# SeanNobel/speech-decoding

Measured on AMD Instinct MI355X. Metric: train segments/sec (Gwilliams2022 208ch x 360, top-10 retrieval acc alongside), higher is better.
Workload: dtype bf16; 1 GPU; Gwilliams2022-shaped MEG: 208 ch x 360 samples, 27 subjects, F=1024, batch 256/GPU, fwd+CLIP loss+top-k+bwd+Adam (BASELINE configs[1]); global_batch=256, seq_len=360, parallelism=dp1

## Files before the change

### include/sd_amd.h

```cpp
#ifndef SD_AMD_H
#define SD_AMD_H
#include <stddef.h>
#include <stdint.h>

#ifdef __cplusplus
extern "C" {
#endif

#define SDA_ABI_VERSION 4
#define SDA_ROW_PAD 16
#define SDA_CH_ALIGN 64

enum { SDA_F32 = 0, SDA_BF16 = 1, SDA_F16 = 2 };

enum { SDA_EPI_GELU = 1,
       SDA_EPI_GLU_BWD = 4,
       SDA_EPI_GLU = 2,
       SDA_CONV_SINGLE_TILE = 4096,
       SDA_CONV_PAIR_TILES = 8192,
       SDA_CONV_ONE_PER_CU = 32768,
       SDA_CONV_FLAT_TILES = 16384,
       SDA_CONV_FLAT_STAGGER = 1024,
       SDA_CONV_WIDE_TILES = 524288,
       SDA_CONV_WAVE_PRIO = 1048576,
// ... 113 lines not shown
int sda_glu_backward_colsum(const void* x, const void* dy, void* dx, float* colsum, float* scratch, int B, int T,
                            int Ch, int dtype, void* stream);
int sda_gelu_backward_colsum(const void* u, const void* dz, void* du, float* colsum, float* scratch, int B, int T,
                             int Cp, int dtype, void* stream);
int sda_glu_backward_colsum_og(const void* out, const void* gate, const void* dy, void* dx, float* colsum, float* scratch,
                               int B, int T, int Ch, int dtype, void* stream);
int sda_colsum(const void* x, float* out, float* scratch , int B, int T,
               int Cp, int dtype, void* stream);

enum { SDA_WGRAD_FLAT_ROWS = 1   };
typedef struct sda_wgrad_args {
  const void* dy;
  const void* x;
  float* g;
  void* out_e;
  const void* sub;
  const float* rscale;
  const float* out_scale;
  const int32_t* perm;
  const int32_t* seg_start;
  int nseg, B, T, Cout_p, Cin_p, KS, dil;
  long dy_pitch, x_pitch, out_pitch;
  long row0, sample_rows;
  long rows_limit;
  long dy_zero_row;
  int co_valid;
  int dtype;
  const float* acc_scale;
  int flags;
} sda_wgrad_args;
int sda_wgrad_gemm(const sda_wgrad_args* a, void* stream);
int sda_wgrad_tile_m(int Cout_p);
int sda_reduce_slabs(const float* src, float* dst, int nslabs, long n, void* stream);
int sda_sim_gemm_ksplit(int M, int N, long K, int dtype);
int sda_sim_gemm(const void* X, const void* W, float* partial, int M, int N, int Np, long K, long pitch, int ksplit, int dtype,
                 void* stream);

int sda_sa_weights_forward(const float* z, const float* cos_t, const float* sin_t, const float* mask,
                           float* W, void* Wp, float* scratch , int D1, int K2,
                           int C, int D1p, int Cp, int dtype, void* stream);
int sda_sa_scratch_floats(int D1, int K2, int C);
int sda_sa_softmax_pack(const float* a, int a_pitch, const float* mask, float* W, void* Wp, int D1, int C, int D1p,
                        int Cp, int dtype, void* stream);
int sda_sa_softmax_backward(const float* dWd, int dwd_pitch, const float* W, const float* mask, float* da,
                            int da_pitch, int D1, int C, void* stream);
int sda_sa_weights_backward(const float* dWd, const float* W, const float* mask, const float* cosT,
                            const float* sinT, float* dz, int D1, int K2, int C, int Cp, void* stream);

int sda_clip_logits_stats(const float* S, long s_pitch, const float* ysq, const float* zsq, const float* temp,
                          float* logits, float* row_max, float* row_sum, float* col_lse, float* diag , float* row_lse ,
                          int Bm, int Bn, int col0, void* stream);
int sda_clip_grad(const float* logits, const float* row_lse, const float* col_lse, const float* ysq,
                  const float* zsq, const float* temp, float inv_norm, int col0, void* G, long g_pitch,
                  float* rscale, float* cscale, float* colpart, float* scalars, int Bm, int Bn, int dtype, void* stream);
int sda_clip_grad_y(const float* logits, const float* row_lse, const float* col_lse, const float* zsq,
                    const float* zsq_all, int nz, int col0, void* Gy, long gy_pitch, int seg, int seg_pitch,
                    float* part, int Bm, int Bn, int dtype, void* stream);
int sda_clip_grad_y_finish(const float* part, int nparts, int Bg, const float* ysq, const float* zsq_all, int nz,
                           const float* temp, float inv_norm, int row0, int nrows, float* rscale_y, float* cscale_y,
                           void* stream);
int sda_clip_dz_supported(int Bm, int Bn, long row_elems, int dtype);
int sda_clip_dz(const void* G, long g_pitch, const void* Y, const void* Z, void* out, const float* cscale, const float* rscale,
                const float* out_scale, int Bm, int Bn, long row_elems, int dtype, void* stream);
int sda_clip_ranks(const float* logits, const float* diag, int32_t* cnt, int Bm, int Bn, int col0, void* stream);
long sda_retrieval_scores_floats(int n, int M, int chunk_cols);
int sda_retrieval_select(const float* S, const float* qsq, const float* csq, const int64_t* labels, int64_t* indices,
// ... 79 lines not shown
```

### speech_decoding_amd/blocks.py

```python
from __future__ import annotations

from dataclasses import dataclass, field
from typing import Dict, Optional

import numpy as np
import torch

from . import lib as L
from . import ops
from .engine import block_dilations, subject_segments

FWD_FLAGS = L.CONV_PAIR_TILES
BWD_FLAGS = L.CONV_WAVE_PRIO


def rows_in(X: torch.Tensor, Cc: int, dtype):
    if X.dtype not in ops.COMPUTE_DTYPES:
        raise L.SdaError(f"input of dtype {X.dtype}: the modules take float32, bfloat16 or float16")
    return ops.rows_of(X, Cc, dtype, ops.new_rows_uninit)


def grad_rows(dY: torch.Tensor, Cc: int, dtype) -> torch.Tensor:
    return ops.rows_of(dY, Cc, dtype, ops.new_rows_uninit)[0]


def _new(B: int, T: int, Cp: int, dtype, dev) -> torch.Tensor:
    return ops.new_rows_uninit(B, T, Cp, dtype, dev)


def _segments(B: int, dy, x):
    nseg = ops.uniform_segment_count(B, ops.wgrad_ntiles(dy.shape[1], x.shape[1], 64))
    return ops.UPLOADER.upload("blocks.seg", ops.uniform_segment_edges(B, nseg), dy.device), nseg


def _wgrad(dy, x, B, T, KS, dil, Cout, Cin, glu_half=0, glu_half_p=0) -> torch.Tensor:
    seg, nseg = _segments(B, dy, x)
    slabs = ops.wgrad_gemm(dy, x, B=B, T=T, KS=KS, dil=dil, seg_start=seg, nseg=nseg, alg_dims=(Cin, Cout), flat_rows=True)
    return ops.reduce_unpack_wgrad(slabs, Cout, Cin, KS, glu_half=glu_half, glu_half_p=glu_half_p)


def _plans(module, dev, build):
    key = (str(dev), module.compute_dtype)
    plans = module.__dict__.setdefault("_block_plans", {})
# ... 59 lines not shown


def _sb_plans(sb):
    D1p = L.pad_channels(sb.D1)

    def build(f, b):
        f.add_weight("sb_w", sb.conv.weight, D1p, D1p)
        f.add_vector("sb_b", sb.conv.bias, D1p)
        f.add_weight("subj_w", sb.subject_layer.weight, D1p, D1p)
        b.add_weight("sb_w", sb.conv.weight, D1p, D1p, mode=1)
        b.add_weight("subj_w", sb.subject_layer.weight, D1p, D1p, mode=1)
        return f, b
    return _plans(sb, sb.conv.weight.device, build)


def _sb_sources(sb) -> Dict[str, torch.Tensor]:
    return {"sb_w": sb.conv.weight.detach(), "sb_b": sb.conv.bias.detach(), "subj_w": sb.subject_layer.weight.detach()}


def subject_block_forward(sb, X: torch.Tensor, sidx: np.ndarray, mask, need_grad: bool, want_subj_grad: bool):
    B, Cc, T = X.shape
    dt, dev, D1, S = sb.compute_dtype, X.device, sb.D1, sb.num_subjects
    D1p = L.pad_channels(D1)
    widx = ops.UPLOADER.upload("blocks.widx", sidx.astype(np.int32), dev)
    Xt, _ = rows_in(X, Cc, dt)
    h_sa, W, Wp = sa_forward(sb.spatial_attention, Xt, B, T, mask, dt)
    pk = _sb_plans(sb)[0].run(_sb_sources(sb))
    h_c = ops.conv_gemm(h_sa, pk["sb_w"], _new(B, T, D1p, dt, dev), B=B, T=T, KS=1, dil=0, bias=pk["sb_b"], alg_dims=(D1, D1))
    y = ops.conv_gemm(h_c, pk["subj_w"], _new(B, T, D1p, dt, dev), B=B, T=T, KS=1, dil=0, widx=widx, alg_dims=(D1, D1))
    if not need_grad:
        return y, None
    c = SBCtx(SACtx(B, T, Xt, W, Wp, mask, X.dtype), h_sa, h_c, widx)
    if want_subj_grad:
        r = ops.subject_slices(B, max(1, int(np.unique(sidx).size)), ops.wgrad_ntiles(D1p, D1p, 64))
        perm, seg = subject_segments(sidx, S, r)
        c.subj = (ops.UPLOADER.upload("blocks.subj_perm", perm, dev), ops.UPLOADER.upload("blocks.subj_seg", seg, dev), r)
    return y, c


def subject_block_backward(sb, c: SBCtx, dY: torch.Tensor, want: Dict[str, bool]) -> Dict[str, torch.Tensor]:
    _check_versions(c)
    B, T, dt, dev = c.sa.B, c.sa.T, sb.compute_dtype, dY.device
    D1, S = sb.D1, sb.num_subjects
    D1p = L.pad_channels(D1)
    g: Dict[str, torch.Tensor] = {}
    if want["subj_w"]:
        perm, seg, r = c.subj
        slabs = ops.wgrad_gemm(dY, c.h_c, B=B, T=T, KS=1, dil=0, perm=perm, seg_start=seg, nseg=r * S, flat_rows=True)
        if r > 1:
            slabs = ops.reduce_slabs(slabs.view(r, -1)).view(S, 1, D1p, D1p)
        g["subj_w"] = ops.unpack_conv_wgrad(slabs, S, D1, D1, 1, D1p, D1p)
    if not (want["sb_w"] or want["sb_b"] or want["z"] or want["X"]):
        return g
    pkT = _sb_plans(sb)[1].run(_sb_sources(sb))
    dh_c = ops.conv_gemm(dY, pkT["subj_w"], _new(B, T, D1p, dt, dev), B=B, T=T, KS=1, dil=0, widx=c.widx, alg_dims=(D1, D1),
                         flags=BWD_FLAGS)
    if want["sb_w"]:
        g["sb_w"] = _wgrad(dh_c, c.h_sa, B, T, 1, 0, D1, D1)
    if want["sb_b"]:
        g["sb_b"] = ops.colsum(dh_c, B, T, ops.reduce_scratch(D1p, dev))[:D1]
    if want["z"] or want["X"]:
        dh_sa = ops.conv_gemm(dh_c, pkT["sb_w"], _new(B, T, D1p, dt, dev), B=B, T=T, KS=1, dil=0, alg_dims=(D1, D1),
                              flags=BWD_FLAGS)
        g["X"], g["z"] = sa_backward(sb.spatial_attention, c.sa, dh_sa, want["X"], want["z"])
    return g


CB_PARAMS = ("c0w", "c0b", "bn0w", "bn0b", "c1w", "c1b", "bn1w", "bn1b", "c2w", "c2b")


def cb_params(cb):
    return [cb.conv0.weight, cb.conv0.bias, cb.batchnorm0.weight, cb.batchnorm0.bias, cb.conv1.weight, cb.conv1.bias,
            cb.batchnorm1.weight, cb.batchnorm1.bias, cb.conv2.weight, cb.conv2.bias]


@dataclass
class CBCtx:
    B: int
    T: int
    x: torch.Tensor
    x_rows: bool
    x_dtype: torch.dtype
    h: list
# ... 112 lines not shown
```

### speech_decoding_amd/csrc/elementwise.hip

```cpp
#include <math.h>

#include "sd_common.h"

namespace sda {

__device__ __forceinline__ void ew_bwd_prio() { __builtin_amdgcn_s_setprio(3); }

struct RowWalk {
  int r, r1, step, T, b, t;
  __device__ RowWalk(int r0, int r1_, int step_, int T_) : r(r0), r1(r1_), step(step_), T(T_) {
    b = r0 / T_;
    t = r0 - b * T_;
  }
  __device__ bool valid() const { return r < r1; }
  __device__ size_t mem_row() const { return (size_t)b * rows_tp(T) + PAD + t; }
  __device__ void next() {
    r += step; t += step;
    while (t >= T) { t -= T; ++b; }
  }
};

struct RowCursor {
  uint32_t off, step, wrap;
  int t, T, RG, n;
// ... 744 lines not shown
  const int RG = nch >= 256 ? 1 : 256 / nch;
  int r0, r1;
  block_rows(B, T, r0, r1);
  for (int c = threadIdx.x; c < RG * nch; c += 256) {
    const int ch = c % nch, rg = c / nch;
    for (RowWalk w(r0 + rg, r1, RG, T); w.valid(); w.next()) {
      const size_t off = w.mem_row() * Cp + ch * CH;
      float uv[CH], d[CH];
      Vec16<E>::load(u + off, uv);
      Vec16<E>::load(dz + off, d);
#pragma unroll
      for (int j = 0; j < CH; j += 2) {
        const f32x2 o = f32x2{d[j], d[j + 1]} * gelu_grad_pair<E>(f32x2{uv[j], uv[j + 1]});
        d[j] = o.x; d[j + 1] = o.y;
      }
      Vec16<E>::store(du + off, d);
    }
  }
}

__global__ void reduce_slabs_kernel(const float* __restrict__ src, float* __restrict__ dst, int nslabs, long n) {
  for (long i = (long)blockIdx.x * blockDim.x + threadIdx.x; i < n; i += (long)gridDim.x * blockDim.x) {
    float s = 0.f;
    int k = 0;
    for (; k + 8 <= nslabs; k += 8) {
      float v[8];
#pragma unroll
      for (int j = 0; j < 8; ++j) v[j] = src[(size_t)(k + j) * n + i];
#pragma unroll
      for (int j = 0; j < 8; ++j) s += v[j];
    }
    for (; k < nslabs; ++k) s += src[(size_t)k * n + i];
    dst[i] = s;
  }
}

static inline int ew_grid(size_t total) {
  size_t g = (total + 255) / 256;
  return (int)(g < 1 ? 1 : (g > 4096 ? 4096 : g));
}

static int red_blocks(int B, int T) {
  long rows = (long)B * T;
  long nb = (rows + 31) / 32;
  if (nb > RED_MAX_BLOCKS) nb = RED_MAX_BLOCKS;
  if (nb < 1) nb = 1;
  return (int)nb;
}

}

using namespace sda;

#define SDA_DISPATCH(dtype, CALL)                                   \
  do {                                                              \
    if ((dtype) == SDA_F32) { using E = float; CALL; }              \
    else if ((dtype) == SDA_BF16) { using E = uint16_t; CALL; }     \
    else if ((dtype) == SDA_F16) { using E = half_t; CALL; }        \
    else { set_error("unknown dtype %d", (int)(dtype)); return -1; } \
  } while (0)

namespace sda {
__global__ __launch_bounds__(256) void zero_pad_rows_kernel(uint4* __restrict__ buf, int B, int Tp, long rows_alloc, int row_vec) {
  const long pad_vecs = (long)B * PAD * row_vec, tail_vecs = (rows_alloc - (long)B * Tp) * row_vec;
  for (long i = (long)blockIdx.x * 256 + threadIdx.x; i < pad_vecs + tail_vecs; i += (long)gridDim.x * 256) {
    long v;
// ... 411 lines not shown
  hipStream_t st = (hipStream_t)stream;
  const int nb = red_blocks(B, T);
  const size_t lds = bwd_colsum_lds(Ch, dtype);
  SDA_DISPATCH(dtype, hipLaunchKernelGGL((bwd_colsum_kernel<E, 1>), dim3(nb), dim3(256), lds, st, (const E*)x,
                                         (const E*)dy, (E*)dx, scratch, B, T, Ch));
  if (colsum) hipLaunchKernelGGL(col_reduce_final_kernel, dim3((Ch + 7) / 8), dim3(256), 0, st, scratch, nb, colsum, colsum + Ch, Ch);
  return check_launch("glu_backward_colsum");
}

extern "C" int sda_glu_backward_colsum_og(const void* out, const void* gate, const void* dy, void* dx, float* colsum,
                                          float* scratch, int B, int T, int Ch, int dtype, void* stream) {
  if (!out || !gate || !dy || !dx || !scratch || Ch % 64 || Ch > 1024 || !fits_u32(B, T, 2L * Ch)) { set_error("glu_backward_colsum_og: bad arguments"); return -1; }
  hipStream_t st = (hipStream_t)stream;
  const int nb = red_blocks(B, T);
  const size_t lds = bwd_colsum_lds(Ch, dtype);
  SDA_DISPATCH(dtype, hipLaunchKernelGGL((bwd_colsum_kernel<E, 2>), dim3(nb), dim3(256), lds, st, (const E*)out,
                                         (const E*)dy, (E*)dx, scratch, B, T, Ch, (const E*)gate));
  if (colsum) hipLaunchKernelGGL(col_reduce_final_kernel, dim3((Ch + 7) / 8), dim3(256), 0, st, scratch, nb, colsum, colsum + Ch, Ch);
  return check_launch("glu_backward_colsum_og");
}

extern "C" int sda_gelu_backward_colsum(const void* u, const void* dz, void* du, float* colsum, float* scratch, int B, int T,
                                        int Cp, int dtype, void* stream) {
  if (!u || !dz || !du || !scratch || Cp % 64 || Cp > 1024 || !fits_u32(B, T, Cp)) { set_error("gelu_backward_colsum: bad arguments"); return -1; }
  hipStream_t st = (hipStream_t)stream;
  const int nb = red_blocks(B, T);
  const size_t lds = bwd_colsum_lds(Cp, dtype);
  SDA_DISPATCH(dtype, hipLaunchKernelGGL((bwd_colsum_kernel<E, 0>), dim3(nb), dim3(256), lds, st, (const E*)u,
                                         (const E*)dz, (E*)du, scratch, B, T, Cp));
  if (colsum) hipLaunchKernelGGL(col_reduce_final_kernel, dim3((Cp + 7) / 8), dim3(256), 0, st, scratch, nb, colsum, (float*)nullptr, Cp);
  return check_launch("gelu_backward_colsum");
}

extern "C" int sda_reduce_slabs(const float* src, float* dst, int nslabs, long n, void* stream) {
  if (!src || !dst || nslabs < 1 || n < 1) { set_error("reduce_slabs: bad arguments"); return -1; }
  hipLaunchKernelGGL(reduce_slabs_kernel, dim3(ew_grid((size_t)n)), dim3(256), 0, (hipStream_t)stream, src, dst, nslabs, n);
  return check_launch("reduce_slabs");
}
```

### speech_decoding_amd/engine.py

```python
from __future__ import annotations

from dataclasses import dataclass, field
from typing import Dict, List, Optional

import ast
import os

import numpy as np
import torch

from . import lib as L
from . import ops


def block_dilations(k: int):
    return 2 ** ((2 * k) % 5), 2 ** ((2 * k + 1) % 5), 2


@dataclass
class EncoderDims:
    C: int
    S: int
    D1: int
    D2: int
    F: int
    K: int

    @property
    def Cp(self): return L.pad_channels(self.C)
    @property
    def D1p(self): return L.pad_channels(self.D1)
    @property
    def D2p(self): return L.pad_channels(self.D2)
    @property
    def F1(self): return 2 * self.D2
    @property
    def F1p(self): return L.pad_channels(2 * self.D2)
    @property
    def Fp(self): return L.pad_channels(self.F)


@dataclass
class EncoderCtx:
    B: int
    T: int
    gen: int
    training: bool
    bufs: Dict[str, torch.Tensor] = field(default_factory=dict)
    packed: Dict[str, torch.Tensor] = field(default_factory=dict)
    bn: Dict[str, tuple] = field(default_factory=dict)
    mask: Optional[torch.Tensor] = None
    widx: Optional[torch.Tensor] = None
    subj_perm: Optional[torch.Tensor] = None
    subj_seg: Optional[torch.Tensor] = None
    subj_slices: int = 1
    W_sa: Optional[torch.Tensor] = None
    packed_T: Dict[str, torch.Tensor] = field(default_factory=dict)
    packed_T_ready: Optional[torch.cuda.Event] = None
    glu_fused: bool = False
    composed: Optional[tuple] = None
    param_grads: bool = True
    x_dtype: Optional[torch.dtype] = None
    W_x: Optional[torch.Tensor] = None


@dataclass
class _Forward:
    eng: "EncoderEngine"
    P: Dict[str, torch.Tensor]
    ctx: EncoderCtx
    dev: torch.device
    main: torch.cuda.Stream
    need_grad: bool
    need_dx: bool
    eps: float
    momentum: float
    k3_flags: int
    count: float
    packed_ready: Optional[torch.cuda.Event] = None
    flip: Dict[int, int] = field(default_factory=dict)

    def rows(self, name, Cp):
        B, T = self.ctx.B, self.ctx.T
        if not self.need_grad:
            name = f"pp{self.flip.setdefault(Cp, 0) % 3}"
            self.flip[Cp] += 1
        return self.eng._rows(name, B, T, Cp, self.dev, "train" if self.need_grad else "eval")

# ... 249 lines not shown
        k3_flags = L.CONV_PAIR_TILES
        if self.flat_forward:
            k3_flags |= L.CONV_FLAT_TILES | L.CONV_FLAT_STAGGER
        f = _Forward(self, P, ctx, dev, torch.cuda.current_stream(dev), need_grad, need_dx, eps, momentum, k3_flags,
                     count=float(B) * T * self.world)

        self._fwd_subjects(f, subject_idxs)
        Xt = ctx.bufs["Xt"] = self._fwd_pack(f, X)
        x = self._fwd_subject_block(f, Xt)
        for k in range(5):
            x = self._fwd_conv_block(f, k, x)
        Zt = self._fwd_projections(f, x)
        if not need_grad:
            ctx.bufs = {"Z": Zt}
            ctx.packed = {}
        return ctx

    def _fwd_subjects(self, f: _Forward, subject_idxs):
        d, ctx = self.d, f.ctx
        B = ctx.B
        sidx = torch.as_tensor(subject_idxs).detach().to("cpu").to(torch.int64).numpy()
        if sidx.shape != (B,):
            raise ValueError("subject_idxs must have shape (B,)")
        if (sidx < 0).any() or (sidx >= d.S).any():
            raise IndexError("subject index out of range")
        up = ops.UPLOADER.upload
        ctx.widx = up(("widx", "train" if f.need_grad else "eval"), sidx.astype(np.int32), f.dev)
        if not (f.need_grad and ctx.param_grads):
            return
        if self.composed:
            ntiles = ops.wgrad_ntiles(d.D2p, d.Cp, 64)
        else:
            ntiles = ops.wgrad_ntiles(d.D1p, d.D1p, 128 if d.D1p % 128 == 0 else 64)
        r = ops.subject_slices(B, max(1, int(np.unique(sidx).size)), ntiles)
        perm, seg = subject_segments(sidx, d.S, r)
        ctx.subj_perm = up("subj_perm", perm, f.dev)
        ctx.subj_seg = up("subj_seg", seg, f.dev)
        ctx.subj_slices = r

    def _fwd_pack(self, f: _Forward, X):
        d, ctx, P = self.d, f.ctx, f.P
        fwd_plan, bwd_plan = self._plans(P, f.dev)
        side = self._side_stream(f.dev) if self.pack_on_side_stream else None
        Xt = f.rows("Xt", d.Cp)
        if side is not None:
            ev = torch.cuda.Event()
            ev.record(f.main)
            side.wait_event(ev)
        with torch.cuda.stream(side):
            ctx.packed.update(fwd_plan.run(P))
            ops.pack_rows(X, Xt, ones_channel=d.C if self.composed else None)
            if side is not None:
                X.record_stream(side)
                f.packed_ready = torch.cuda.Event()
                f.packed_ready.record(side)
            if f.need_grad:
                ctx.packed_T = bwd_plan.run(P)
                if side is not None:
                    ctx.packed_T_ready = torch.cuda.Event()
                    ctx.packed_T_ready.record(side)
        return Xt

    def _fwd_subject_block(self, f: _Forward, Xt):
        d, ctx, P, dev = self.d, f.ctx, f.P, f.dev
        B, T, pk = ctx.B, ctx.T, ctx.packed
        composed = self.composed
        ctx.W_sa, Wp = ops.sa_weights_forward(P["z"], P["cos"], P["sin"], ctx.mask, d.D1p, d.Cp,
                                              torch.float32 if composed else self.dtype, fwd_table=P.get("sa_tab_f"))
        if not composed:
            ctx.W_x = Wp if f.need_dx else None
            if f.packed_ready is not None:
# ... 191 lines not shown
                                              allreduce=self._allreduce if sync else None, tile_stats=tstats)
            if sync and pg:
                both = dgam._base if dgam._base is not None else torch.stack([dgam, dbet])
                if b.side is not None:
                    both.record_stream(b.side)
                scaled = b.on_side(lambda: both / world)
                dgam, dbet = scaled[0], scaled[1]
            if pg:
                grads[bnp + "w"], grads[bnp + "b"] = dgam[: d.D2], dbet[: d.D2]
                grads[f"b{k}.c{j}b"] = null_bias[2 * k + j] if ctx.training else ops.bias_grad(ops.colsum(dh, B, T, scratch), d.D2)
            src, ci, ci_p = (bufs[f"b{k}.a0"], d.D2, d.D2p) if j == 1 else (bufs[f"x{k}"], cin, cin_p)
            key = f"b{k}.c{j}w"
            res = dh if (j == 1 or k > 0) else None
            out = b.tmp("da", d.D2p) if j == 1 else b.tmp("dxB" if k % 2 == 0 else "dxA", ci_p)
            if k == 0 and j == 0 and ctx.composed is not None and ctx.x_dtype is None:
                da1 = None
            else:
                da1, tstats = b.dgrad(dh, key, out, 3, dil[j], res=res,
                                      bn=(bufs[f"b{k}.h0"], ctx.bn[f"b{k}.bn0"][2]) if j == 1 else None)
            grads[key] = b.wgrad(dh, src, 3, dil[j], d.D2, ci)
        b.flush([f"b{k}.c2w", f"b{k}.c2b", f"b{k}.c1w", f"b{k}.c1b", f"b{k}.bn1w", f"b{k}.bn1b",
                 f"b{k}.c0w", f"b{k}.c0b", f"b{k}.bn0w", f"b{k}.bn0b"])
        return da1, dh

    def _bwd_subject_composed(self, b: _Backward, dx, dh0, w0cat):
        d, ctx, P, grads = self.d, b.ctx, b.P, b.grads
        B, T, dev = b.B, b.T, b.dev
        if ctx.x_dtype is not None:
            grads["X"] = ops.input_grad(dx, ctx.W_x, ctx.widx, B, d.C, T, ctx.x_dtype)
        if not b.pg:
            return
        Wd, T1aug, Ws = ctx.composed
        W0cat, w0cat_ready = w0cat
        r = ctx.subj_slices
        M = ops.wgrad_gemm(dh0, ctx.bufs["Xt"], B=B, T=T, KS=3, dil=block_dilations(0)[0], perm=ctx.subj_perm,
                           seg_start=ctx.subj_seg, nseg=r * d.S, flat_rows=True)
        if r > 1:
            M = ops.reduce_slabs(M.view(r, -1))
        if w0cat_ready is not None:
            self._wait("W0cat copy (side stream)", b.main, w0cat_ready)
        G = ops.param_gemm(W0cat.view(d.D1, 3 * d.D2p), M.view(d.S, 3 * d.D2p, d.Cp)[:, :, : d.C + 1])
        grads["subj_w"] = b.on_side(lambda: ops.param_gemm(G, T1aug.t()).view(d.S, d.D1, d.D1, 1))
        part = ops.param_gemm(Ws.transpose(1, 2), G)
        dT1f = ops.reduce_slabs(part.view(d.S, -1)).view(d.D1, d.C + 1)
        dT1 = dT1f[:, : d.C]
        grads["sb_b"], grads["sb_w"] = b.on_side(lambda: (
            ops.copy3d(torch.empty(d.D1, dtype=torch.float32, device=dev), dT1f[:, d.C]),
            ops.param_gemm(dT1, Wd.t()).unsqueeze(-1)))
        dWd = ops.param_gemm(P["sb_w"][..., 0].t(), dT1)
        grads["z"] = ops.sa_weights_backward(dWd, ctx.W_sa, ctx.mask, P["cosT"], P["sinT"], P["z"].shape[1],
                                             bwd_table=P.get("sa_tab_b"))

    def _bwd_subject_three_conv(self, b: _Backward, dhs):
        d, ctx, P, grads, pg = self.d, b.ctx, b.P, b.grads, b.pg
        B, T, bufs = b.B, b.T, ctx.bufs

        def subj_wgrad():
            r = ctx.subj_slices
            slabs = ops.wgrad_gemm(dhs, bufs["h_c"], B=B, T=T, KS=1, dil=0, perm=ctx.subj_perm, seg_start=ctx.subj_seg,
                                   nseg=r * d.S, flat_rows=True)
            if r > 1:
                slabs = ops.reduce_slabs(slabs.view(r, -1)).view(d.S, 1, d.D1p, d.D1p)
            return ops.unpack_conv_wgrad(slabs, d.S, d.D1, d.D1, 1, d.D1p, d.D1p)
        if pg:
            grads["subj_w"] = b.on_side(subj_wgrad)
        dh_c, _ = b.dgrad(dhs, "subj_w", b.tmp("dh_c", d.D1p), 1, 0, widx=ctx.widx)
        if pg:
            grads["sb_w"] = b.wgrad(dh_c, bufs["h_sa"], 1, 0, d.D1, d.D1)
            grads["sb_b"] = ops.bias_grad(ops.colsum(dh_c, B, T, b.scratch), d.D1)
        dh_sa, _ = b.dgrad(dh_c, "sb_w", b.tmp("dh_sa", d.D1p), 1, 0)
        if ctx.x_dtype is not None:
            grads["X"] = ops.input_grad(dh_sa, ctx.W_x, None, B, d.C, T, ctx.x_dtype)
        if not pg:
            return
        perm, seg, nseg = self._uniform_segments(B, ops.wgrad_ntiles(d.D1p, d.Cp, 64), b.dev)
        dWd = ops.reduce_slabs(ops.wgrad_gemm(dh_sa, bufs["Xt"], B=B, T=T, KS=1, dil=0, perm=perm, seg_start=seg, nseg=nseg))
        grads["z"] = ops.sa_weights_backward(dWd, ctx.W_sa, ctx.mask, P["cosT"], P["sinT"], P["z"].shape[1],
                                             bwd_table=P.get("sa_tab_b"))


def subject_segments(sidx: np.ndarray, S: int, r: int):
    order = np.argsort(sidx, kind="stable").astype(np.int32)
    bounds = np.searchsorted(sidx[order], np.arange(S + 1)).astype(np.int64)
    lo, hi = bounds[:-1], bounds[1:]
    cuts = [lo + ((hi - lo) * j) // r for j in range(r + 1)]
    seg = np.empty(r * S + 1, dtype=np.int32)
    parts, pos = [], 0
    for j in range(r):
        for s in range(S):
            a_, b_ = int(cuts[j][s]), int(cuts[j + 1][s])
            seg[j * S + s] = pos
            parts.append(order[a_:b_])
            pos += b_ - a_
    seg[r * S] = pos
    perm = np.concatenate(parts).astype(np.int32) if parts else order
# ... 89 lines not shown
```

### speech_decoding_amd/lib.py

```python
from __future__ import annotations

import ctypes as C
import os

_HERE = os.path.dirname(os.path.abspath(__file__))
LIB_PATH = os.path.join(_HERE, "libsdamd.so")

ABI_VERSION = 4
F32, BF16, F16 = 0, 1, 2
ROW_PAD = 16
CH_ALIGN = 64
EPI_GELU, EPI_GLU, EPI_GLU_BWD = 1, 2, 4
EPI_GELU_BWD, EPI_ROW_SUMSQ, EPI_BN_STORE_DG = 65536, 131072, 262144
CONV_SINGLE_TILE, CONV_PAIR_TILES, CONV_FLAT_TILES, CONV_ONE_PER_CU = 4096, 8192, 16384, 32768
CONV_WAVE_PRIO = 1048576
CONV_FLAT_STAGGER = 1024
CONV_WIDE_TILES = 524288
WGRAD_FLAT_ROWS = 1

vp, i32, i64, f32, f64 = C.c_void_p, C.c_int, C.c_long, C.c_float, C.c_double


class ConvArgs(C.Structure):
    _fields_ = [("x", vp), ("w", vp), ("bias", vp), ("res", vp), ("y", vp), ("y_pre", vp), ("widx", vp),
# ... 54 lines not shown
    "sda_pack_vector": (i32, [vp, vp, i32, i32, i32, i32, vp]),
    "sda_unpack_conv_wgrad": (i32, [vp, vp, i32, i32, i32, i32, i32, i32, i32, i32, vp]),
    "sda_unpack_vector": (i32, [vp, vp, i32, i32, i32, i32, vp]),
    "sda_conv_gemm": (i32, [C.POINTER(ConvArgs), vp]),
    "sda_conv_n_t_tiles": (i32, [i32]),
    "sda_conv_tile_co": (i32, [i32, i32, i32]),
    "sda_conv_stats_rows": (i32, [i32, i32, i32, i32, i32]),
    "sda_bn_finalize": (i32, [vp, i32, f64, vp, vp, f32, f32, vp, vp, vp, vp, vp, vp, vp, i32, i32, i32, vp, vp]),
    "sda_reduce_stats": (i32, [vp, i32, vp, vp, i32, vp]),
    "sda_bn_gelu_backward_from_stats": (i32, [vp, i32, vp, vp, vp, vp, vp, vp, i32, f64, vp, vp, vp, vp, i32, i32, i32, i32, vp]),
    "sda_bn_gelu_backward_from_stats_dg": (i32, [vp, i32, vp, vp, vp, vp, vp, vp, i32, f64, vp, vp, vp, vp, i32, i32, i32, i32, vp]),
    "sda_bn_gelu_forward": (i32, [vp, vp, vp, vp, i32, i32, i32, i32, vp]),
    "sda_bn_gelu_backward_reduce": (i32, [vp, vp, vp, vp, vp, vp, i32, vp, vp, vp, i32, i32, i32, i32, vp]),
    "sda_bn_gelu_backward_apply": (i32, [vp, vp, vp, vp, vp, vp, i32, vp, vp, f64, vp, vp, i32, i32, i32, i32, vp]),
    "sda_bn_gelu_backward_apply_dg": (i32, [vp, vp, vp, vp, vp, vp, i32, vp, vp, f64, vp, vp, i32, i32, i32, i32, vp]),
    "sda_reduce_scratch_floats": (i32, [i32]),
    "sda_glu_forward": (i32, [vp, vp, i32, i32, i32, i32, vp]),
    "sda_glu_backward": (i32, [vp, vp, vp, i32, i32, i32, i32, vp]),
    "sda_gelu_backward": (i32, [vp, vp, vp, i32, i32, i32, i32, vp]),
    "sda_reduce_scratch_rows": (i32, [i32, i32]),
    "sda_glu_backward_colsum": (i32, [vp, vp, vp, vp, vp, i32, i32, i32, i32, vp]),
    "sda_w2v_conv0": (i32, [vp, i64, vp, vp, vp, vp, vp, i32, i32, i32, i32, i32, f32, i32, vp]),
    "sda_layernorm_rows": (i32, [vp, vp, vp, vp, i32, i32, i32, f32, i32, i32, vp]),
    "sda_w2v_group_split": (i32, [vp, vp, i32, i32, i32, i32, i32, i64, i32, i32, vp]),
    "sda_w2v_group_merge_add": (i32, [vp, vp, vp, i32, i32, i32, i32, i32, i64, vp, i32, i32, vp]),
    "sda_w2v_attention": (i32, [vp, vp, vp, vp, i32, i32, i32, i64, i64, i64, f32, i32, vp]),
    "sda_splitk_epilogue": (i32, [vp, i32, vp, vp, vp, i32, i32, i32, i32, vp]),
    "sda_w2v_mean4": (i32, [vp, vp, vp, vp, vp, i32, i32, i32, i32, vp]),
    "sda_glu_backward_colsum_og": (i32, [vp, vp, vp, vp, vp, vp, i32, i32, i32, i32, vp]),
    "sda_gelu_backward_colsum": (i32, [vp, vp, vp, vp, vp, i32, i32, i32, i32, vp]),
    "sda_colsum": (i32, [vp, vp, vp, i32, i32, i32, i32, vp]),
    "sda_wgrad_gemm": (i32, [C.POINTER(WgradArgs), vp]),
    "sda_wgrad_tile_m": (i32, [i32]),
    "sda_reduce_slabs": (i32, [vp, vp, i32, i64, vp]),
    "sda_sa_weights_forward": (i32, [vp, vp, vp, vp, vp, vp, vp, i32, i32, i32, i32, i32, i32, vp]),
    "sda_sa_scratch_floats": (i32, [i32, i32, i32]),
    "sda_sa_softmax_pack": (i32, [vp, i32, vp, vp, vp, i32, i32, i32, i32, i32, vp]),
    "sda_sa_softmax_backward": (i32, [vp, i32, vp, vp, vp, i32, i32, i32, vp]),
    "sda_sa_weights_backward": (i32, [vp, vp, vp, vp, vp, vp, i32, i32, i32, i32, vp]),
    "sda_clip_logits_stats": (i32, [vp, i64, vp, vp, vp, vp, vp, vp, vp, vp, vp, i32, i32, i32, vp]),
    "sda_clip_grad": (i32, [vp, vp, vp, vp, vp, vp, f32, i32, vp, i64, vp, vp, vp, vp, i32, i32, i32, vp]),
    "sda_clip_grad_y": (i32, [vp, vp, vp, vp, vp, i32, i32, vp, i64, i32, i32, vp, i32, i32, i32, vp]),
    "sda_clip_grad_y_finish": (i32, [vp, i32, i32, vp, vp, i32, vp, f32, i32, i32, vp, vp, vp]),
    "sda_collate_rows": (i32, [vp, vp, i64, i32, i32, f32, i32, vp]),
    "sda_collate_windows": (i32, [vp, vp, vp, i32, i32, i32, i32, f32, i32, vp]),
    "sda_robust_stats_scratch_bytes": (i64, [i64]),
    "sda_robust_stats": (i32, [vp, i64, i64, i32, i64, i64, vp, vp, vp, i64, vp]),
    "sda_scale_clamp_rows": (i32, [vp, vp, i64, i64, i32, i64, i64, vp, vp, f32, i32, vp]),
    "sda_gather_baseline_windows": (i32, [vp, vp, vp, i32, i32, i32, i32, vp]),
    "sda_clip_ranks": (i32, [vp, vp, vp, i32, i32, i32, vp]),
    "sda_retrieval_scores_floats": (i64, [i32, i32, i32]),
    "sda_retrieval_select": (i32, [vp, vp, vp, vp, vp, vp, vp, i32, i32, i32, i32, vp]),
    "sda_retrieval_class_reduce": (i32, [vp, vp, vp, vp, vp, vp, vp, i64, i32, i32, i32, i32, f32, i32, vp]),
    "sda_retrieval_pool_rows": (i32, [vp, i64, vp, vp, vp, i64, i32, i32, i32, vp]),
    "sda_clip_dz_supported":(i32, [i32, i32, i64, i32]),
    "sda_clip_dz": (i32, [vp, i64, vp, vp, vp, vp, vp, vp, i32, i32, i64, i32, vp]),
    "sda_param_gemm": (i32, [C.POINTER(PgemmArgs), vp]),
    "sda_zero_pad_rows": (i32, [vp, i32, i32, i32, i32, vp]),
    "sda_scalar_mul": (i32, [vp, vp, vp, i32, vp]),
    "sda_fill_zero": (i32, [vp, i64, vp]),
    "sda_gather_samples": (i32, [vp, vp, vp, i32, i64, vp]),
    "sda_clip_merge_rows": (i32, [vp, i32, i32, vp, vp, vp]),
    "sda_copy3d": (i32, [vp, i64, i64, i64, vp, i64, i64, i64, i32, i32, i32, vp]),
    "sda_mse_forward": (i32, [vp, i32, i32, vp, i32, i32, i32, i32, i32, i32, vp, vp, vp]),
    "sda_mse_backward": (i32, [vp, i32, i32, vp, i32, i32, i32, i32, i32, i32, vp, vp, vp, vp]),
    "sda_input_grad": (i32, [vp, i64, vp, vp, i32, i32, i32, i32, i32, i32, i32, vp, i32, vp]),
# ... 50 lines not shown
```

### speech_decoding_amd/ops.py

```python
from __future__ import annotations

import ctypes as C
from typing import Optional

import numpy as np
import torch

from . import lib as L

_DT = {torch.float32: L.F32, torch.bfloat16: L.BF16, torch.float16: L.F16}
COMPUTE_DTYPES = tuple(_DT)


def dt_code(dtype: torch.dtype) -> int:
    try:
        return _DT[dtype]
    except KeyError:
        raise L.SdaError(f"unsupported compute dtype {dtype}; use torch.float32, torch.bfloat16 or torch.float16")


def _p(t: Optional[torch.Tensor]):
    return None if t is None else t.data_ptr()


# ... 638 lines not shown
    return cs


def colsum(x, B, T, scratch):
    out = torch.empty(x.shape[1], dtype=torch.float32, device=x.device)
    L.check(L.load().sda_colsum(_p(x), _p(out), _p(scratch), B, T, x.shape[1], dt_code(x.dtype), _st()), "colsum")
    return out


WGRAD_TARGET_WGS = 256


def wgrad_tile_m(Cout_p: int) -> int:
    return L.load().sda_wgrad_tile_m(Cout_p)


def wgrad_ntiles(Cout_p: int, Cin_p: int, tile_n: int = 64) -> int:
    return (Cout_p // wgrad_tile_m(Cout_p)) * (Cin_p // tile_n)


def splitk_tile_co(Np: int) -> int:
    return 160 if Np % 160 == 0 else (128 if Np % 128 == 0 else 64)


def uniform_segment_count(B: int, ntiles: int) -> int:
    nseg = 8 * max(1, round(WGRAD_TARGET_WGS / (8 * max(1, ntiles))))
    return int(min(B, nseg)) if B >= 8 else int(max(1, min(B, nseg)))


def uniform_segment_edges(B: int, nseg: int) -> np.ndarray:
    return np.floor(np.linspace(0, B, nseg + 1)).astype(np.int32)


def subject_slices(B: int, present: int, ntiles: int) -> int:
    return int(max(1, min(max(1, B // present), round(WGRAD_TARGET_WGS / max(1, ntiles * present)))))


def bias_grad(cs, C, glu_half=0, glu_half_p=0):
    if glu_half == 0 or glu_half_p == glu_half:
        return cs[:C]
    return unpack_vector(cs, C, glu_half, glu_half_p)


def wgrad_args(dy, x, *, B, T, Cout_p, Cin_p, KS, dil, dy_pitch, x_pitch, rows_limit, dtype, flags=0, g=None, perm=None,
               seg_start=None, nseg=1, row0=L.ROW_PAD, sample_rows=None, dy_zero_row=0, out_e=None, out_pitch=0, co_valid=0,
               sub=None, rscale=None, acc_scale=None, out_scale=None) -> L.WgradArgs:
    return L.WgradArgs(dy, x, g, out_e, sub, rscale, out_scale, perm, seg_start, nseg, B, T, Cout_p, Cin_p, KS, dil, dy_pitch, x_pitch,
                       out_pitch, row0, L.rows_tp(T) if sample_rows is None else sample_rows, rows_limit, dy_zero_row, co_valid, dtype,
                       acc_scale, flags)


def wgrad_gemm(dy, x, *, B, T, KS, dil, perm=None, seg_start=None, nseg=1, alg_dims=None, flat_rows=False):
    g = torch.empty((nseg, KS, dy.shape[1], x.shape[1]), dtype=torch.float32, device=x.device)
    if nseg > 1 and seg_start is None:
        raise L.SdaError("wgrad_gemm: nseg > 1 needs seg_start")
    a = wgrad_args(_p(dy), _p(x), B=B, T=T, Cout_p=dy.shape[1], Cin_p=x.shape[1], KS=KS, dil=dil, dy_pitch=dy.shape[1],
                   x_pitch=x.shape[1], rows_limit=x.shape[0], dtype=dt_code(x.dtype), g=_p(g), perm=_p(perm), seg_start=_p(seg_start),
                   nseg=nseg, flags=L.WGRAD_FLAT_ROWS if flat_rows else 0)
    cin, cout = alg_dims if alg_dims is not None else (x.shape[1], dy.shape[1])
    _launch("wgrad_gemm", lambda: (("wgrad_gemm", str(x.dtype).replace("torch.", ""), wgrad_tile_m(dy.shape[1]), KS),
                                   2.0 * B * T * KS * cin * cout), L.load().sda_wgrad_gemm, a, "wgrad_gemm")
    return g


def reduce_slabs(slabs: torch.Tensor) -> torch.Tensor:
    n = slabs[0].numel()
# ... 301 lines not shown
```

Before: 37580 segments/s.

## Split subject wgrad segments by per-subject counts and reduce slab groups

Subject-specific weight-gradient segmentation used to split every subject into the same number of slices r. It now picks a per-subject split count from that subject's sample count, so all segments stay under a common size bound within a work-group budget. A new grouped slab-reduction kernel sums each subject's variable number of partial slabs. This targets load imbalance and idle work in the per-subject wgrad GEMM. The cost is an extra reduce launch whenever segments are split, plus more host-side planning.

```diff
diff --git a/include/sd_amd.h b/include/sd_amd.h
--- a/include/sd_amd.h
+++ b/include/sd_amd.h
@@ -169,6 +169,7 @@
 int sda_wgrad_gemm(const sda_wgrad_args* a, void* stream);
 int sda_wgrad_tile_m(int Cout_p);
 int sda_reduce_slabs(const float* src, float* dst, int nslabs, long n, void* stream);
+int sda_reduce_slab_groups(const float* src, float* dst, const int32_t* first, int ngroups, long n, void* stream);
 int sda_sim_gemm_ksplit(int M, int N, long K, int dtype);
 int sda_sim_gemm(const void* X, const void* W, float* partial, int M, int N, int Np, long K, long pitch, int ksplit, int dtype,
                  void* stream);
diff --git a/speech_decoding_amd/blocks.py b/speech_decoding_amd/blocks.py
--- a/speech_decoding_amd/blocks.py
+++ b/speech_decoding_amd/blocks.py
@@ -8,7 +8,7 @@
 
 from . import lib as L
 from . import ops
-from .engine import block_dilations, subject_segments
+from .engine import block_dilations
 
 FWD_FLAGS = L.CONV_PAIR_TILES
 BWD_FLAGS = L.CONV_WAVE_PRIO
@@ -134,9 +134,9 @@
         return y, None
     c = SBCtx(SACtx(B, T, Xt, W, Wp, mask, X.dtype), h_sa, h_c, widx)
     if want_subj_grad:
-        r = ops.subject_slices(B, max(1, int(np.unique(sidx).size)), ops.wgrad_ntiles(D1p, D1p, 64))
-        perm, seg = subject_segments(sidx, S, r)
-        c.subj = (ops.UPLOADER.upload("blocks.subj_perm", perm, dev), ops.UPLOADER.upload("blocks.subj_seg", seg, dev), r)
+        perm, seg, first = ops.subject_segment_plan(sidx, S, ops.wgrad_ntiles(D1p, D1p, 64))
+        c.subj = (ops.UPLOADER.upload("blocks.subj_perm", perm, dev), ops.UPLOADER.upload("blocks.subj_seg", seg, dev),
+                  None if first is None else ops.UPLOADER.upload("blocks.subj_first", first, dev))
     return y, c
 
 
@@ -147,10 +147,9 @@
     D1p = L.pad_channels(D1)
     g: Dict[str, torch.Tensor] = {}
     if want["subj_w"]:
-        perm, seg, r = c.subj
-        slabs = ops.wgrad_gemm(dY, c.h_c, B=B, T=T, KS=1, dil=0, perm=perm, seg_start=seg, nseg=r * S, flat_rows=True)
-        if r > 1:
-            slabs = ops.reduce_slabs(slabs.view(r, -1)).view(S, 1, D1p, D1p)
+        perm, seg, first = c.subj
+        slabs = ops.wgrad_gemm(dY, c.h_c, B=B, T=T, KS=1, dil=0, perm=perm, seg_start=seg, nseg=seg.numel() - 1, flat_rows=True)
+        slabs = ops.reduce_slab_groups(slabs, first, S)
         g["subj_w"] = ops.unpack_conv_wgrad(slabs, S, D1, D1, 1, D1p, D1p)
     if not (want["sb_w"] or want["sb_b"] or want["z"] or want["X"]):
         return g
diff --git a/speech_decoding_amd/csrc/elementwise.hip b/speech_decoding_amd/csrc/elementwise.hip
--- a/speech_decoding_amd/csrc/elementwise.hip
+++ b/speech_decoding_amd/csrc/elementwise.hip
@@ -800,6 +800,24 @@
     }
     for (; k < nslabs; ++k) s += src[(size_t)k * n + i];
     dst[i] = s;
+  }
+}
+
+__global__ void reduce_slab_groups_kernel(const float* __restrict__ src, float* __restrict__ dst, const int32_t* __restrict__ first, long n) {
+  const int k0 = first[blockIdx.y], k1 = first[blockIdx.y + 1];
+  float* __restrict__ out = dst + (size_t)blockIdx.y * n;
+  for (long i = (long)blockIdx.x * blockDim.x + threadIdx.x; i < n; i += (long)gridDim.x * blockDim.x) {
+    float s = 0.f;
+    int k = k0;
+    for (; k + 4 <= k1; k += 4) {
+      float v[4];
+#pragma unroll
+      for (int j = 0; j < 4; ++j) v[j] = src[(size_t)(k + j) * n + i];
+#pragma unroll
+      for (int j = 0; j < 4; ++j) s += v[j];
+    }
+    for (; k < k1; ++k) s += src[(size_t)k * n + i];
+    out[i] = s;
   }
 }
 
@@ -1277,6 +1295,13 @@
   return check_launch("gelu_backward_colsum");
 }
 
+extern "C" int sda_reduce_slab_groups(const float* src, float* dst, const int32_t* first, int ngroups, long n, void* stream) {
+  if (!src || !dst || !first || ngroups < 1 || ngroups > 65535 || n < 1) { set_error("reduce_slab_groups: bad arguments"); return -1; }
+  const int gx = ew_grid((size_t)n);
+  hipLaunchKernelGGL(reduce_slab_groups_kernel, dim3(gx < 1024 ? gx : 1024, ngroups), dim3(256), 0, (hipStream_t)stream, src, dst, first, n);
+  return check_launch("reduce_slab_groups");
+}
+
 extern "C" int sda_reduce_slabs(const float* src, float* dst, int nslabs, long n, void* stream) {
   if (!src || !dst || nslabs < 1 || n < 1) { set_error("reduce_slabs: bad arguments"); return -1; }
   hipLaunchKernelGGL(reduce_slabs_kernel, dim3(ew_grid((size_t)n)), dim3(256), 0, (hipStream_t)stream, src, dst, nslabs, n);
diff --git a/speech_decoding_amd/engine.py b/speech_decoding_amd/engine.py
--- a/speech_decoding_amd/engine.py
+++ b/speech_decoding_amd/engine.py
@@ -53,7 +53,8 @@
     widx: Optional[torch.Tensor] = None
     subj_perm: Optional[torch.Tensor] = None
     subj_seg: Optional[torch.Tensor] = None
-    subj_slices: int = 1
+    subj_first: Optional[torch.Tensor] = None
+    subj_nseg: int = 0
     W_sa: Optional[torch.Tensor] = None
     packed_T: Dict[str, torch.Tensor] = field(default_factory=dict)
     packed_T_ready: Optional[torch.cuda.Event] = None
@@ -369,11 +370,10 @@
             ntiles = ops.wgrad_ntiles(d.D2p, d.Cp, 64)
         else:
             ntiles = ops.wgrad_ntiles(d.D1p, d.D1p, 128 if d.D1p % 128 == 0 else 64)
-        r = ops.subject_slices(B, max(1, int(np.unique(sidx).size)), ntiles)
-        perm, seg = subject_segments(sidx, d.S, r)
+        perm, seg, first = ops.subject_segment_plan(sidx, d.S, ntiles)
         ctx.subj_perm = up("subj_perm", perm, f.dev)
-        ctx.subj_seg = up("subj_seg", seg, f.dev)
-        ctx.subj_slices = r
+        tables = up("subj_seg", seg if first is None else np.concatenate([seg, first]), f.dev)
+        ctx.subj_seg, ctx.subj_first, ctx.subj_nseg = tables[: seg.size], (None if first is None else tables[seg.size:]), seg.size - 1
 
     def _fwd_pack(self, f: _Forward, X):
         d, ctx, P = self.d, f.ctx, f.P
@@ -631,11 +631,9 @@
             return
         Wd, T1aug, Ws = ctx.composed
         W0cat, w0cat_ready = w0cat
-        r = ctx.subj_slices
         M = ops.wgrad_gemm(dh0, ctx.bufs["Xt"], B=B, T=T, KS=3, dil=block_dilations(0)[0], perm=ctx.subj_perm,
-                           seg_start=ctx.subj_seg, nseg=r * d.S, flat_rows=True)
-        if r > 1:
-            M = ops.reduce_slabs(M.view(r, -1))
+                           seg_start=ctx.subj_seg, nseg=ctx.subj_nseg, flat_rows=True)
+        M = ops.reduce_slab_groups(M, ctx.subj_first, d.S)
         if w0cat_ready is not None:
             self._wait("W0cat copy (side stream)", b.main, w0cat_ready)
         G = ops.param_gemm(W0cat.view(d.D1, 3 * d.D2p), M.view(d.S, 3 * d.D2p, d.Cp)[:, :, : d.C + 1])
@@ -655,11 +653,9 @@
         B, T, bufs = b.B, b.T, ctx.bufs
 
         def subj_wgrad():
-            r = ctx.subj_slices
             slabs = ops.wgrad_gemm(dhs, bufs["h_c"], B=B, T=T, KS=1, dil=0, perm=ctx.subj_perm, seg_start=ctx.subj_seg,
-                                   nseg=r * d.S, flat_rows=True)
-            if r > 1:
-                slabs = ops.reduce_slabs(slabs.view(r, -1)).view(d.S, 1, d.D1p, d.D1p)
+                                   nseg=ctx.subj_nseg, flat_rows=True)
+            slabs = ops.reduce_slab_groups(slabs, ctx.subj_first, d.S)
             return ops.unpack_conv_wgrad(slabs, d.S, d.D1, d.D1, 1, d.D1p, d.D1p)
         if pg:
             grads["subj_w"] = b.on_side(subj_wgrad)
diff --git a/speech_decoding_amd/lib.py b/speech_decoding_amd/lib.py
--- a/speech_decoding_amd/lib.py
+++ b/speech_decoding_amd/lib.py
@@ -110,6 +110,7 @@
     "sda_colsum": (i32, [vp, vp, vp, i32, i32, i32, i32, vp]),
     "sda_wgrad_gemm": (i32, [C.POINTER(WgradArgs), vp]),
     "sda_wgrad_tile_m": (i32, [i32]),
+    "sda_reduce_slab_groups": (i32, [vp, vp, vp, i32, i64, vp]),
     "sda_reduce_slabs": (i32, [vp, vp, i32, i64, vp]),
     "sda_sa_weights_forward": (i32, [vp, vp, vp, vp, vp, vp, vp, i32, i32, i32, i32, i32, i32, vp]),
     "sda_sa_scratch_floats": (i32, [i32, i32, i32]),
diff --git a/speech_decoding_amd/ops.py b/speech_decoding_amd/ops.py
--- a/speech_decoding_amd/ops.py
+++ b/speech_decoding_amd/ops.py
@@ -694,6 +694,45 @@
     return np.floor(np.linspace(0, B, nseg + 1)).astype(np.int32)
 
 
+SUBJECT_TARGET_WGS = 2 * WGRAD_TARGET_WGS
+
+
+def subject_segment_plan(sidx, S: int, ntiles: int):
+    sidx = np.asarray(sidx).astype(np.int64)
+    order = np.argsort(sidx, kind="stable").astype(np.int32)
+    counts = np.bincount(sidx, minlength=S).astype(np.int64)
+    budget = max(1, SUBJECT_TARGET_WGS // max(1, ntiles))
+    nmax = int(counts.max()) if counts.size else 0
+    bound = max(1, nmax)
+    for cand in range(1, nmax):
+        if int(((counts + cand - 1) // cand).sum()) <= budget:
+            bound = cand
+            break
+    if bound >= nmax:
+        return order, np.concatenate([[0], np.cumsum(counts)]).astype(np.int32), None
+    k = (counts + bound - 1) // bound
+    first = np.concatenate([[0], np.cumsum(k)]).astype(np.int32)
+    lo = np.concatenate([[0], np.cumsum(counts)])
+    seg = np.empty(int(first[-1]) + 1, dtype=np.int32)
+    for s in range(S):
+        for j in range(int(k[s])):
+            seg[first[s] + j] = lo[s] + (counts[s] * j) // k[s]
+    seg[-1] = sidx.size
+    return order, seg, first
+
+
+def reduce_slab_groups(slabs: torch.Tensor, first: torch.Tensor, ngroups: int) -> torch.Tensor:
+    if first is None:
+        if slabs.shape[0] != ngroups:
+            raise L.SdaError("reduce_slab_groups: one slab per group expected")
+        return slabs
+    if first.numel() != ngroups + 1 or first.dtype != torch.int32:
+        raise L.SdaError("reduce_slab_groups: first must be int32 [ngroups + 1]")
+    out = torch.empty((ngroups,) + tuple(slabs.shape[1:]), dtype=torch.float32, device=slabs.device)
+    L.check(L.load().sda_reduce_slab_groups(_p(slabs), _p(out), _p(first), ngroups, slabs[0].numel(), _st()), "reduce_slab_groups")
+    return out
+
+
 def subject_slices(B: int, present: int, ntiles: int) -> int:
     return int(max(1, min(max(1, B // present), round(WGRAD_TARGET_WGS / max(1, ntiles * present)))))
 
```

Measured after the change: 37500 segments/s. About the same (-0.2%).
